# Abolfazlmsl/Oriented-Object-Detection

Hardware: AMD Instinct MI355X
Metric: 416px tiles/sec (whole node), YOLOv11n-OBB 3ch (higher is better)
Workload: dtype f32; 1 GPU; YOLOv11n-OBB 3ch 416x416 tiled inference, single-scale (BASELINE configs[1]): forward + decode + ProbIoU NMS + border filter + per-tile merge + final polygon-IoU merge; step_pipelining=True, nc=12, weights=synthetic seeded, cls bias -8 (no checkpoint offline), final_detections=12170

## Files before the change

### include/obbhip.h

```cpp
#ifndef OBBHIP_H
#define OBBHIP_H

#include <stddef.h>
#include <stdint.h>

#ifdef __cplusplus
extern "C" {
#endif

#define OBB_OK 0
#define OBB_ERR_INVALID (-1)
#define OBB_ERR_HIP (-2)
#define OBB_ERR_STATE (-3)
#define OBB_ERR_FORMAT (-4)

typedef struct obb_ctx obb_ctx;
typedef void *obb_stream_t;

int obb_version(void);
int obb_ctx_create(int device, obb_ctx **out);
int obb_ctx_destroy(obb_ctx *ctx);
const char *obb_last_error(const obb_ctx *ctx);

int obb_set_option(obb_ctx *ctx, const char *key, int64_t value);
// ... 102 lines not shown
int obb_headconv_bwd_geometry(int64_t N, int32_t cin, int32_t cout, int32_t out[4]);
int obb_stemconv_fwd_u8(obb_ctx *ctx, const uint8_t *x, const float *w, int32_t B, int32_t H, int32_t W, int32_t cin, int32_t cout, uint16_t *z,
                        obb_stream_t s);
int obb_stemconv_wgrad_u8(obb_ctx *ctx, const uint8_t *x, const uint16_t *dz, int32_t B, int32_t H, int32_t W, int32_t cin, int32_t cout,
                          float *dw, obb_stream_t s);
int obb_stemconv_wgrad_geometry(int32_t B, int32_t H, int32_t W, int32_t cin, int32_t cout, int32_t out[4]);
int obb_attn_fwd_bf16(obb_ctx *ctx, const uint16_t *qkv, int32_t B, int32_t N, int32_t nh, uint16_t *out, float *lse, obb_stream_t s);
int obb_attn_bwd_bf16(obb_ctx *ctx, const uint16_t *qkv, const uint16_t *out, const float *lse, const uint16_t *dout, const uint16_t *dv_add,
                      int32_t B, int32_t N, int32_t nh, uint16_t *dqkv, obb_stream_t s);
int obb_add_bf16(obb_ctx *ctx, const uint16_t *a, const uint16_t *b, int64_t n, uint16_t *out, obb_stream_t s);
int obb_chanwin_bf16(obb_ctx *ctx, const uint16_t *src, int32_t Cs, int32_t s0, const uint16_t *add, int32_t Ca, int32_t a0, int64_t npix, int32_t n,
                     uint16_t *dst, int32_t Cd, int32_t d0, obb_stream_t s);

int obb_model_load(obb_ctx *ctx, const void *blob_host, size_t bytes);
int obb_model_unload(obb_ctx *ctx, int32_t slot);
int obb_model_info(const obb_ctx *ctx, int32_t h, int32_t w, int32_t *nc, int32_t *ch, int32_t *anchors, int32_t *nconv);
int obb_forward(obb_ctx *ctx, const uint8_t *tiles, int32_t B, int32_t h, int32_t w, float *head, obb_stream_t s);
int obb_forward_gate(obb_ctx *ctx, const uint8_t *tiles, int32_t B, int32_t h, int32_t w, float *head, float *cmax, obb_stream_t s);
int obb_debug_plan(obb_ctx *ctx, int32_t h, int32_t w, char *buf_host, int64_t buf_bytes, int64_t *needed);
int obb_debug_pack_1x1(int32_t form, const float *w, int32_t cout, int32_t cin, int32_t c0, int32_t nc, float *out, int64_t max_floats,
                       int64_t *needed, int32_t *tiling_host);
int obb_debug_activation(obb_ctx *ctx, int32_t h, int32_t w, int32_t B, const char *name, float *out, int64_t max_elems,
                         int64_t *n_elems, int32_t *shape_hwc_host, obb_stream_t s);
int obb_decode_nms(obb_ctx *ctx, const float *head, int32_t B, int32_t h, int32_t w, float conf_thres, float iou_thres,
                   int32_t max_det, float *out, int32_t *count, obb_stream_t s);
int obb_decode_nms_gate(obb_ctx *ctx, const float *head, const float *cmax, int32_t B, int32_t h, int32_t w, float conf_thres, float iou_thres,
                        int32_t max_det, float *det, int32_t *count, obb_stream_t s);
int obb_decode_nms_full(obb_ctx *ctx, const float *head, int32_t B, int32_t h, int32_t w, float conf_thres, float iou_thres,
                        int32_t max_det, float *out, int32_t *count, obb_stream_t s);
int obb_decode(obb_ctx *ctx, const float *head, int32_t B, int32_t h, int32_t w, float *pred, obb_stream_t s);
int obb_probiou_nms(obb_ctx *ctx, const float *boxes, const float *scores, int64_t n, float iou_thres, int32_t *order,
                    uint8_t *keep, obb_stream_t s);
int obb_results(obb_ctx *ctx, const float *det, const float *lb, int64_t n, float *xywhr, float *pts, obb_stream_t s);

int obb_probiou_loss(obb_ctx *ctx, const float *pred, const float *target, const float *weight, int64_t n, float target_scores_sum,
                     float *loss, float *grad_pred, obb_stream_t s);

int obb_tile_labels(obb_ctx *ctx, const double *labels, int64_t n, const int32_t *rects, int32_t ntiles, double min_fraction, uint8_t *mask,
                    double *out, obb_stream_t s);

int obb_dfl_loss(obb_ctx *ctx, const float *pred_dist, const float *target_ltrb, const float *weight, int64_t n, int32_t reg_max,
                 float target_scores_sum, float *loss, float *grad_pred, obb_stream_t s);
int obb_bce_loss(obb_ctx *ctx, const float *logits, const float *targets, int64_t n, float target_scores_sum, float *loss, float *grad_logits,
                 obb_stream_t s);

int obb_crit_decode(obb_ctx *ctx, const void *const *box, int32_t box_bf16, const float *const *cls, const float *const *angle, const int32_t *H,
// ... 51 lines not shown
```

### oriented-object-detection_amd/_lib.py

```python
import ctypes as C
import os

_HERE = os.path.dirname(os.path.abspath(__file__))
SO_PATH = os.path.join(_HERE, "libobbhip.so")
if os.environ.get("OBB_LIB"):
    import sys
    SO_PATH = os.environ["OBB_LIB"]
    sys.stderr.write("oriented_object_detection_amd: OBB_LIB is set -- loading the DIAGNOSTIC library %s instead of the product build\n" % SO_PATH)
_lib = None

c_dp, c_fp, c_ip, c_lp, c_bp = (C.POINTER(C.c_double), C.POINTER(C.c_float), C.POINTER(C.c_int32),
                                C.POINTER(C.c_int64), C.POINTER(C.c_uint8))
_V = C.c_void_p

SIGNATURES = {
    "obb_version": [],
    "obb_ctx_create": [C.c_int, C.POINTER(_V)],
    "obb_ctx_destroy": [_V],
    "obb_last_error": [_V],
    "obb_set_option": [_V, C.c_char_p, C.c_int64],
    "obb_poly_iou_pairs": [_V, _V, _V, C.c_int64, _V, _V],
    "obb_poly_iou_matrix": [_V, _V, _V, C.c_int64, _V, _V, C.c_int64, _V, _V],
    "obb_points_in_quads": [_V, _V, _V, C.c_int64, _V, _V, C.c_int64, _V, _V],
    "obb_build_multich": [_V, _V, C.c_int32, C.c_int32, C.c_int32, _V, _V],
# ... 39 lines not shown
    "obb_headconv_fwd_bf16": [_V, _V, _V, _V, C.c_int64, C.c_int32, C.c_int32, _V, _V],
    "obb_headconv_bwd_bf16": [_V, _V, _V, _V, C.c_int64, C.c_int32, C.c_int32, _V, _V, _V, _V],
    "obb_headconv_bwd_geometry": [C.c_int64, C.c_int32, C.c_int32, c_ip],
    "obb_stemconv_fwd_u8": [_V, _V, _V, C.c_int32, C.c_int32, C.c_int32, C.c_int32, C.c_int32, _V, _V],
    "obb_stemconv_wgrad_u8": [_V, _V, _V, C.c_int32, C.c_int32, C.c_int32, C.c_int32, C.c_int32, _V, _V],
    "obb_stemconv_wgrad_geometry": [C.c_int32, C.c_int32, C.c_int32, C.c_int32, C.c_int32, c_ip],
    "obb_bn_fwd_bf16": [_V, _V, C.c_int64, C.c_int32, _V, _V, C.c_float, C.c_float, _V, _V, _V, _V, _V, C.c_int32, _V],
    "obb_bn_bwd_bf16": [_V, _V, _V, C.c_int64, C.c_int32, _V, _V, _V, _V, _V, _V, _V, C.c_int32, _V],
    "obb_attn_fwd_bf16": [_V, _V, C.c_int32, C.c_int32, C.c_int32, _V, _V, _V],
    "obb_attn_bwd_bf16": [_V, _V, _V, _V, _V, _V, C.c_int32, C.c_int32, C.c_int32, _V, _V],
    "obb_add_bf16": [_V, _V, _V, C.c_int64, _V, _V],
    "obb_chanwin_bf16": [_V, _V, C.c_int32, C.c_int32, _V, C.c_int32, C.c_int32, C.c_int64, C.c_int32, _V, C.c_int32, C.c_int32, _V],
    "obb_gather_tiles": [_V, _V, C.c_int32, C.c_int32, C.c_int32, _V, C.c_int32, C.c_int32, _V, _V],
    "obb_letterbox": [_V, _V, C.c_int32, C.c_int32, C.c_int32, C.c_int32, C.c_int32, C.c_int32, C.c_int32, C.c_int32, _V,
                      C.c_int32, C.c_int32, _V],
    "obb_model_load": [_V, _V, C.c_size_t],
    "obb_model_unload": [_V, C.c_int32],
    "obb_model_info": [_V, C.c_int32, C.c_int32, c_ip, c_ip, c_ip, c_ip],
    "obb_forward": [_V, _V, C.c_int32, C.c_int32, C.c_int32, _V, _V],
    "obb_forward_gate": [_V, _V, C.c_int32, C.c_int32, C.c_int32, _V, _V, _V],
    "obb_debug_plan": [_V, C.c_int32, C.c_int32, C.c_char_p, C.c_int64, c_lp],
    "obb_debug_pack_1x1": [C.c_int32, _V, C.c_int32, C.c_int32, C.c_int32, C.c_int32, _V, C.c_int64, c_lp, c_ip],
    "obb_debug_activation": [_V, C.c_int32, C.c_int32, C.c_int32, C.c_char_p, _V, C.c_int64, c_lp, c_ip, _V],
    "obb_decode_nms": [_V, _V, C.c_int32, C.c_int32, C.c_int32, C.c_float, C.c_float, C.c_int32, _V, _V, _V],
    "obb_decode_nms_gate": [_V, _V, _V, C.c_int32, C.c_int32, C.c_int32, C.c_float, C.c_float, C.c_int32, _V, _V, _V],
    "obb_decode_nms_full": [_V, _V, C.c_int32, C.c_int32, C.c_int32, C.c_float, C.c_float, C.c_int32, _V, _V, _V],
    "obb_decode": [_V, _V, C.c_int32, C.c_int32, C.c_int32, _V, _V],
    "obb_probiou_nms": [_V, _V, _V, C.c_int64, C.c_float, _V, _V, _V],
    "obb_results": [_V, _V, _V, C.c_int64, _V, _V, _V],
    "obb_probiou_loss": [_V, _V, _V, _V, C.c_int64, C.c_float, _V, _V, _V],
    "obb_tile_labels": [_V, _V, C.c_int64, _V, C.c_int32, C.c_double, _V, _V, _V],
    "obb_dfl_loss": [_V, _V, _V, _V, C.c_int64, C.c_int32, C.c_float, _V, _V, _V],
    "obb_bce_loss": [_V, _V, _V, C.c_int64, C.c_float, _V, _V, _V],
    "obb_crit_decode": [_V, _V, C.c_int32, _V, _V, c_ip, c_ip, C.c_int32, C.c_int32, _V, _V, _V, _V, _V],
    "obb_crit_loss": [_V, _V, C.c_int32, _V, _V, c_ip, c_ip, C.c_int32, C.c_int32, _V, _V, _V, c_fp, _V, _V, _V, _V, _V, _V],
    "obb_sgd_step": [_V, _V, _V, _V, C.c_int64, C.c_float, C.c_float, C.c_float, C.c_int32, C.c_int32, _V],
    "obb_adamw_step": [_V, _V, _V, _V, _V, C.c_int64, C.c_int64, C.c_float, C.c_double, C.c_double, C.c_float, C.c_float, _V],
    "obb_grad_sumsq_partials": [c_lp, C.c_int32, c_lp],
    "obb_grad_sumsq": [_V, _V, c_lp, C.c_int32, _V, C.c_int64, _V],
    "obb_clip_coef": [_V, _V, C.c_int64, C.c_double, _V, _V],
    "obb_sgd_step_multi": [_V, _V, _V, _V, c_lp, c_fp, c_fp, C.c_int32, C.c_float, C.c_int32, C.c_int32, _V, _V],
    "obb_adamw_step_multi": [_V, _V, _V, _V, _V, c_lp, c_fp, c_fp, C.c_int32, C.c_int64, C.c_double, C.c_double, C.c_float, _V, _V],
    "obb_grad_accumulate": [_V, _V, _V, c_lp, C.c_int32, C.c_int32, _V],
    "obb_ema_update": [_V, _V, _V, c_lp, C.c_int32, C.c_double, _V],
    "obb_aug_tiles": [_V, _V, C.c_int32, C.c_int32, C.c_int32, _V, C.c_int32, C.c_int32, C.c_int32, _V, _V],
    "obb_aug_labels": [_V, _V, _V, C.c_int32, C.c_int32, _V, C.c_int32, C.c_int32, C.c_double, C.c_double, C.c_double, C.c_int32, _V, _V, _V, _V, _V],
# ... 40 lines not shown
```

### oriented-object-detection_amd/csrc/ctx.h

```cpp
#pragma once
#include <hip/hip_runtime.h>

#include <cstdarg>
#include <cstdint>
#include <cstdio>
#include <map>
#include <memory>
#include <string>
#include <vector>

#include "../../include/obbhip.h"

namespace obb {
struct Model;
struct EngineOpts {
    bool tail = true, tail16 = true, bneck = true, bneck_cv2 = true, c3kimg = true, dwpw = true, upfold = true, stem = true, front = true, pair = true, hmerge = true,
         sppf_fuse = true, attn_mfma = true, xtile = true, nitile = true, nc2 = true, blk32 = true, c3k2f = true, pw32 = true, upacc = true, graph = true;
    int fwd_split = 0 , microbatch = 1024;
};
}

struct obb_ctx {
    int device = 0;
    std::string err;
    struct Slot { void *p = nullptr; size_t bytes = 0; };
    std::vector<Slot> ws;
    std::shared_ptr<obb::Model> model;
    std::map<int, std::shared_ptr<obb::Model>> slots;
    int slot = 0;
    bool opt_f16 = true;
    bool opt_f32 = false;
    obb::EngineOpts opt;
    void *workspace(int slot, size_t bytes);
    ~obb_ctx();
};

namespace obb {
int set_error(obb_ctx *ctx, int code, const char *fmt, ...);
extern thread_local std::string g_tls_error;

// ... 20 lines not shown
```

### oriented-object-detection_amd/csrc/engine.hip

```cpp
#include <algorithm>
#include <cmath>
#include <cstdlib>
#include <cstring>

#include "plan.h"

namespace obb {

static int ensure_capacity(obb_ctx *ctx, Plan &P, int B) {
    if (B <= P.cap) return OBB_OK;
    int cap = std::max(B, 1);
    int64_t off = 0;
    for (Buf &b : P.bufs) {
        b.off = off;
        if (b.virt) continue;
        off += ((int64_t)cap * b.per_img() * (b.f32 ? 4 : 2) + 255) / 256 * 256;
    }
    void *slab = nullptr;
    OBB_HIP(ctx, hipDeviceSynchronize());
    P.drop_graphs();
    if (P.slab) { (void)hipFree(P.slab); P.slab = nullptr; P.cap = 0; }
    OBB_HIP(ctx, hipMalloc(&slab, (size_t)off + 256));
    P.slab = slab;
    P.cap = cap;
// ... 206 lines not shown
                                    float *__restrict__ dst, int blk, int64_t ps) {
    int64_t i = (int64_t)blockIdx.x * 256 + threadIdx.x;
    int64_t total = (int64_t)B * npix_per_img * C;
    if (i >= total) return;
    int c = (int)(i % C) + co;
    int64_t pix = (i / C) % npix_per_img;
    int64_t b = i / ((int64_t)C * npix_per_img);
    dst[i] = HX<F16>::one(blk > 0 ? src[(int64_t)(c / blk) * ps + b * bs + pix * blk + c % blk] : src[b * bs + pix * cs + c]);
}

__global__ void k_f32_slice_copy(const float *__restrict__ src, int64_t bs, int cs, int co, int C, int64_t npix_per_img, int B, float *__restrict__ dst, int blk) {
    int64_t i = (int64_t)blockIdx.x * 256 + threadIdx.x;
    if (i >= (int64_t)B * npix_per_img * C) return;
    int c = (int)(i % C) + co;
    int64_t pix = (i / C) % npix_per_img;
    int64_t b = i / ((int64_t)C * npix_per_img);
    dst[i] = blk > 0 ? src[b * bs + (int64_t)(c / blk) * npix_per_img * blk + pix * blk + c % blk] : src[b * bs + pix * cs + c];
}

static bool *switch_of(obb_ctx *ctx, const std::string &k) {
    struct { const char *key; bool *flag; } sw[] = {
        {"tail", &ctx->opt.tail}, {"tail16", &ctx->opt.tail16}, {"bneck", &ctx->opt.bneck}, {"bneck_cv2", &ctx->opt.bneck_cv2},
        {"c3kimg", &ctx->opt.c3kimg}, {"dwpw", &ctx->opt.dwpw}, {"upfold", &ctx->opt.upfold}, {"stem", &ctx->opt.stem}, {"front", &ctx->opt.front}, {"pair", &ctx->opt.pair},
        {"hmerge", &ctx->opt.hmerge}, {"sppf_fuse", &ctx->opt.sppf_fuse}, {"attn_mfma", &ctx->opt.attn_mfma}, {"xtile", &ctx->opt.xtile}, {"nitile", &ctx->opt.nitile}, {"nc2", &ctx->opt.nc2}, {"blk32", &ctx->opt.blk32}, {"c3k2f", &ctx->opt.c3k2f}, {"pw32", &ctx->opt.pw32}, {"upacc", &ctx->opt.upacc}, {"graph", &ctx->opt.graph}};
    for (auto &e : sw)
        if (k == e.key) return e.flag;
    return nullptr;
}

}

using namespace obb;

extern "C" {

int obb_model_load(obb_ctx *ctx, const void *blob_host, size_t bytes) {
    OBB_REQUIRE(ctx, ctx && blob_host && bytes > 0, "obb_model_load: bad arguments");
    OBB_HIP(ctx, hipSetDevice(ctx->device));
    OBB_HIP(ctx, hipDeviceSynchronize());
    std::shared_ptr<Model> M(new Model());
    M->blob.assign((const char *)blob_host, (const char *)blob_host + bytes);
    int rc = parse_blob(ctx, *M);
    if (rc) return rc;
    M->f16 = ctx->opt_f16;
    M->f32 = ctx->opt_f32;
    M->o = ctx->opt;
    M->o.hmerge = M->o.tail && M->o.hmerge;
// ... 163 lines not shown
                const int ni = (!op.one_d && ctx->model->o.nitile) ? conv_ni_supported(L) : 1;
                snprintf(line, sizeof line, "conv %s k%d s%d cin%d cout%d out%dx%d TH%d TW%d MF%d NF%d CK%d NI%d gx%d gy%d lds%d macs%.0f\n", op.name.c_str(), L.ks,
                         L.stride, L.cin, L.cout, op.Ho, op.Wo, ni > 1 ? op.Ho : L.TH, ni > 1 ? op.Wo : L.TW, L.MF, L.NF, L.CK, ni, grid_x, grid_y, (int)conv_lds_bytes(L), op.macs);
                break;
            }
            case OP_DW: snprintf(line, sizeof line, "dwconv %s c%d out%dx%d macs%.0f\n", op.name.c_str(), op.in.C, op.Ho, op.Wo, op.macs); break;
            case OP_C3KIMG: snprintf(line, sizeof line, "c3kimg %s c%d out%dx%d macs%.0f\n", op.name.c_str(), op.in.C, op.Ho, op.Wo, op.macs); break;
            case OP_DWPW: snprintf(line, sizeof line, "dwpw %s c%d tail%d out%dx%d macs%.0f\n", op.name.c_str(), op.dwpw.cin, op.dwpw.tail_cout, op.Ho, op.Wo, op.macs); break;
            case OP_BNECK: snprintf(line, sizeof line, "bneck %s c%d co%d out%dx%d rows4 macs%.0f\n", op.name.c_str(), op.bneck.C, op.bneck.CO, op.Ho, op.Wo, op.macs); break;
            case OP_SPPF: snprintf(line, sizeof line, "pool %s c%d out%dx%d x3 macs0\n", op.name.c_str(), op.in.C, op.Ho, op.Wo); break;
            case OP_POOL: snprintf(line, sizeof line, "pool %s c%d out%dx%d macs0\n", op.name.c_str(), op.in.C, op.Ho, op.Wo); break;
            case OP_UP: snprintf(line, sizeof line, "upsample %s c%d out%dx%d macs0\n", op.name.c_str(), op.in.C, op.Ho, op.Wo); break;
            case OP_PW32:
                snprintf(line, sizeof line, "pw32 %s k1 s1 cin%d cout%d out%dx%d waves%d raw%d lds%d macs%.0f\n", op.name.c_str(), op.pw32.cin, op.pw32.cout, op.Ho, op.Wo,
                         op.pw32.cin * 256 <= 80 * 1024 ? 8 : 16, op.pw32.raw ? 1 : 0, op.pw32.cin * 256, op.macs);
                break;
            case OP_C3K2F32: {
                int th, tw;
                c3k2f32_tile(op.H, op.W, th, tw);
                snprintf(line, sizeof line, "c3k2f32 %s c%d co%d out%dx%d TH%d TW%d macs%.0f\n", op.name.c_str(), op.c3k2f.C, op.c3k2f.CO, op.Ho, op.Wo, th, tw, op.macs);
                break;
            }
            case OP_STEM32:
                snprintf(line, sizeof line, "stem32 %s k3 s2 cin%d cout%d out%dx%d rows%d macs%.0f\n", op.name.c_str(), op.stem32.cin, op.stem32.cout, op.Ho, op.Wo, 4, op.macs);
                break;
            case OP_STEM:
                snprintf(line, sizeof line, "stem %s k3 s2 cin%d cout%d out%dx%d rows%d macs%.0f\n", op.name.c_str(), op.stem.cin, op.stem.cout, op.Ho, op.Wo, 4, op.macs);
                break;
            case OP_FRONT: snprintf(line, sizeof line, "front %s cin%d out%dx%d macs%.0f\n", op.name.c_str(), op.front.cin, op.Ho, op.Wo, op.macs); break;
            case OP_ATTN: snprintf(line, sizeof line, "attn %s N%d nh%d macs%.0f\n", op.name.c_str(), op.N, op.nh, op.macs); break;
        }
        out += line;
    }
    snprintf(line, sizeof line, "total_macs %.0f bytes_per_img %lld nbufs %zu nops %zu\n", P->macs_per_img, (long long)P->bytes_per_img, P->bufs.size(),
             P->ops.size());
    out += line;
    *needed = (int64_t)out.size() + 1;
    if (buf && buf_bytes >= *needed) memcpy(buf, out.c_str(), out.size() + 1);
    return OBB_OK;
}

int obb_debug_activation(obb_ctx *ctx, int32_t h, int32_t w, int32_t B, const char *name, float *out, int64_t max_elems,
                         int64_t *n_elems, int32_t *shape_hwc_host, obb_stream_t s) {
    OBB_REQUIRE(ctx, ctx && name && n_elems, "obb_debug_activation: bad arguments");
    Plan *P = nullptr;
    int rc = get_plan(ctx, h, w, &P);
    if (rc) return rc;
// ... 2 lines not shown
    OBB_REQUIRE(ctx, B <= P->cap, "obb_debug_activation: run obb_forward with B >= %d first", B);
    const Slice &sl = it->second;
    const Buf &b = P->bufs[sl.buf];
    int64_t n = (int64_t)B * b.H * b.W * sl.C;
    *n_elems = n;
    if (shape_hwc_host) { shape_hwc_host[0] = b.H; shape_hwc_host[1] = b.W; shape_hwc_host[2] = sl.C; }
    if (!out) return OBB_OK;
    OBB_REQUIRE(ctx, max_elems >= n, "obb_debug_activation: output too small (%lld < %lld)", (long long)max_elems, (long long)n);
    const int64_t hw = (int64_t)b.H * b.W;
    const int64_t d_bs = b.blk > 0 ? hw * b.blk : b.per_img(), d_ps = b.blk > 0 ? (int64_t)P->cap * hw * b.blk : 0;
    if (b.f32)
        hipLaunchKernelGGL(k_f32_slice_copy, dim3((unsigned)cdiv(n, 256)), dim3(256), 0, (hipStream_t)s, (const float *)b.p, (int64_t)b.per_img(), b.C, sl.co, sl.C, hw,
                           B, out, b.blk32);
    else if (ctx->model->f16)
        hipLaunchKernelGGL(k_half_slice_to_f32<true>, dim3((unsigned)cdiv(n, 256)), dim3(256), 0, (hipStream_t)s, (const bf16_t *)b.p, d_bs, b.C,
                           sl.co, sl.C, hw, B, out, b.blk, d_ps);
    else
        hipLaunchKernelGGL(k_half_slice_to_f32<false>, dim3((unsigned)cdiv(n, 256)), dim3(256), 0, (hipStream_t)s, (const bf16_t *)b.p, d_bs, b.C,
                           sl.co, sl.C, hw, B, out, b.blk, d_ps);
    OBB_LAUNCH_CHECK(ctx);
    return OBB_OK;
}

}
```

### oriented-object-detection_amd/csrc/f32path.h

```cpp
#pragma once
#include <hip/hip_runtime.h>

#include <cstdint>
#include <vector>

#include "tensorref.h"

namespace obb {

struct Conv32Tiling { int TH, TW, CK, WC, MFM, NI, NC; };

struct Conv32Launch {
    TensorRef in, out, res;
    const float *wpk = nullptr;
    const float *bias = nullptr;
    const float *lut = nullptr;
    int B = 0, Hin = 0, Win = 0, Hout = 0, Wout = 0;
    int cin = 0, cout = 0, ks = 1, stride = 1, act = 1, in_u8 = 0, flip_bgr = 0;
    int out_hw = 0;
    TensorRef in2;
    int up_c = 0, up_W = 0, up_HW = 0;
    TensorRef acc_init;
    const float *tail_w = nullptr;
    const float *tail_b = nullptr;
// ... 5 lines not shown
    int TH = 1, TW = 208, CK = 16, WC = 4, MFM = 7;
    int dw = 0, dw_act = 1;
    int NI = 1;
    int tiles_y = 1, tiles_x = 1;
    int NC = 1;
    int xtile = 1;
    void set_tiling(const Conv32Tiling &t) { TH = t.TH; TW = t.TW; CK = t.CK; WC = t.WC; MFM = t.MFM; NI = t.NI; NC = t.NC; }
};

Conv32Tiling plan_conv32(int ks, int stride, int cin, int cout, int Hout, int Wout, bool in_u8, bool vcat = false, bool nc2 = false);
bool conv32_tail_supported(const Conv32Tiling &t, int cout1, int cout2);
Conv32Tiling plan_dwpw32(int cin, int cout, int H, int W);
std::vector<float> pack_dwpw32_weights(const float *pw_oihw, int cout, int cin, const float *dw_c9, const float *dw_bias, const Conv32Tiling &t);
std::vector<float> pack_conv32_weights(const float *w_oihw, int cout, int cin, int ks, const Conv32Tiling &t, const int *cout_perm, bool in_u8);
size_t conv32_lds_bytes(const Conv32Launch &L);
hipError_t launch_conv32(const Conv32Launch &L, hipStream_t st);

struct Stem32Launch {
    const uint8_t *in = nullptr;
    TensorRef out;
    const float *wpk = nullptr;
    const float *bias = nullptr, *lut = nullptr;
    int B = 0, Hin = 0, Win = 0, cin = 3, cout = 16, act = 1;
};
bool stem32_supported(int cin, int cout, int ks, int stride, int Hin, int Win);
std::vector<float> pack_stem32_weights(const float *w_oihw, int cout, int cin, bool flip_bgr);
hipError_t launch_stem32(const Stem32Launch &L, hipStream_t st);

hipError_t launch_dwconv3_f32(const TensorRef &in, const TensorRef &out, const TensorRef &res, const float *w9c, const float *bias, int B, int H, int W,
                              int C, int act, hipStream_t st);
hipError_t launch_maxpool5_f32(const TensorRef &in, const TensorRef &out, int B, int H, int W, int C, hipStream_t st);
hipError_t launch_upsample2_f32(const TensorRef &in, const TensorRef &out, int B, int H, int W, int C, hipStream_t st);
hipError_t launch_sppf_pools_f32(const TensorRef &cat, int B, int H, int W, int C, hipStream_t st);
hipError_t launch_attention_f32(const TensorRef &qkv, const TensorRef &out, int B, int N, int nh, int kd, int hd, bool use_mfma, hipStream_t st);

}
```

### oriented-object-detection_amd/csrc/f32path.hip

```cpp
#include "f32path.h"
#include "c32geom.h"
#include "c32params.h"
#include "launchcfg.h"

#include <algorithm>
#include <cmath>
#include <cstdlib>
#include <cstring>

namespace obb {

typedef __attribute__((ext_vector_type(4))) float f32x4;
typedef __attribute__((ext_vector_type(4))) unsigned int u32x4;

__device__ __forceinline__ float silu32(float x) { return x * __builtin_amdgcn_rcpf(1.0f + __expf(-x)); }

template <int KS, int MFM, int WC, int NW, bool IN_U8, bool VCAT, int TAIL, bool DW = false, int NC = 1, bool BLK = false, bool AINIT = false>
__global__ __launch_bounds__(NW * 64, NW / 2) void k_conv_f32(const C32Params P) {
    static_assert(NW == c32::kNW, "the planner and the launch checks size tiles for c32::kNW waves");
    static_assert(!AINIT || (KS == 1 && NC == 2 && !VCAT), "accumulator init: the 1-D 1x1 two-fragment form only");
    static_assert(NC == 1 || (NC == 2 && TAIL == 0 && !DW && !IN_U8), "two cout fragments per wave: plain / VCAT forms only");
    extern __shared__ __attribute__((aligned(16))) char smem[];
    constexpr int SKS = DW ? 3 : KS;
    constexpr int NT = NW * 64, WP = NW / WC, PAD = SKS / 2;
    const int tid = threadIdx.x, lane = tid & 63;
    const int wave = __builtin_amdgcn_readfirstlane(tid >> 6);
    const int g = lane >> 4, pl = lane & 15;
    const int wc = wave % WC, wp = wave / WC;
    const int xcd = blockIdx.x & 7, lin = blockIdx.x >> 3;
    const int cb = lin % P.ncb;
    int t = (lin / P.ncb) * 8 + xcd;
// ... 639 lines not shown
            for (int nf = 0; nf < NF; ++nf) {
                acc0[nf] = __builtin_amdgcn_mfma_f32_16x16x4f32(wA[nf][t], b0[t], acc0[nf], 0, 0, 0);
                acc1[nf] = __builtin_amdgcn_mfma_f32_16x16x4f32(wA[nf][t], b1[t], acc1[nf], 0, 0, 0);
            }
        }
#pragma unroll
        for (int h = 0; h < 2; ++h) {
            if (h == 1 && !two) break;
            float *op = orow + (int64_t)(16 * (f0 + h) + j) * P.out_cs;
#pragma unroll
            for (int nf = 0; nf < NF; ++nf) {
                const f32x4 a = h ? acc1[nf] : acc0[nf];
                float v[4] = {a[0] + bv[nf].x, a[1] + bv[nf].y, a[2] + bv[nf].z, a[3] + bv[nf].w};
                if (P.act) {
#pragma unroll
                    for (int q = 0; q < 4; ++q) v[q] = silu32(v[q]);
                }
                *reinterpret_cast<float4 *>(op + nf * 16) = make_float4(v[0], v[1], v[2], v[3]);
            }
        }
    }
}

static int stem32_rs(int Win, int cin) { return (4 + Win * cin + 3) & ~3; }

bool stem32_supported(int cin, int cout, int ks, int stride, int Hin, int Win) {
    if (ks != 3 || stride != 2 || (cin != 3 && cin != 4) || (cout != 16 && cout != 32)) return false;
    if (Hin % 8 || Win % 32) return false;
    return (size_t)(9 * stem32_rs(Win, cin) + 256) * 4 <= 64 * 1024 && 9 * Win * cin / 4 <= 16 * 256;
}

hipError_t launch_stem32(const Stem32Launch &L, hipStream_t st) {
    if (!stem32_supported(L.cin, L.cout, 3, 2, L.Hin, L.Win) || L.out.cpb || (L.out.cs & 3) || (L.out.co & 3) || !L.lut) return hipErrorInvalidValue;
    Stem32Params P;
    P.in = L.in; P.in_bs = (int64_t)L.Hin * L.Win * L.cin;
    P.out = (float *)L.out.p; P.out_bs = L.out.bs; P.out_cs = L.out.cs; P.out_co = L.out.co;
    P.wA = L.wpk; P.bias = L.bias; P.lut = L.lut;
    P.Hin = L.Hin; P.Win = L.Win; P.Hout = L.Hin / 2; P.Wout = L.Win / 2; P.act = L.act; P.RS = stem32_rs(L.Win, L.cin);
    const size_t lds = (size_t)(9 * P.RS + 256) * 4;
    const dim3 grid((unsigned)(L.B * (P.Hout / 4)));
    if (L.cin == 3 && L.cout == 16) hipLaunchKernelGGL((k_stem_f32<3, 1>), grid, dim3(256), lds, st, P);
    else if (L.cin == 4 && L.cout == 16) hipLaunchKernelGGL((k_stem_f32<4, 1>), grid, dim3(256), lds, st, P);
    else if (L.cin == 3 && L.cout == 32) hipLaunchKernelGGL((k_stem_f32<3, 2>), grid, dim3(256), lds, st, P);
    else hipLaunchKernelGGL((k_stem_f32<4, 2>), grid, dim3(256), lds, st, P);
    return hipGetLastError();
}

__global__ __launch_bounds__(256) void k_dwconv3_f32(TensorRef in, TensorRef out, TensorRef res, const float *__restrict__ w, const float *__restrict__ bias,
                                                    int B, int H, int W, int C, int act) {
    const int c4n = C >> 2;
    const int64_t idx = (int64_t)blockIdx.x * 256 + threadIdx.x;
    if (idx >= (int64_t)B * H * W * c4n) return;
    const int c4 = (int)(idx % c4n);
    const int64_t pix = idx / c4n;
    const int x = (int)(pix % W), y = (int)((pix / W) % H), b = (int)(pix / ((int64_t)W * H));
    const float *ip = (const float *)in.p + (int64_t)b * in.bs + in.co + c4 * 4;
// ... 344 lines not shown
```

### oriented-object-detection_amd/csrc/netplan.hip

```cpp
#include <algorithm>
#include <cmath>
#include <cstring>

#include "plan.h"

namespace obb {

#pragma pack(push, 1)
struct BlobHeader { char magic[4]; uint32_t version, nrec; int32_t nc, ch; float width, depth; int32_t max_ch, reg_max; char scale[8]; };
struct BlobRec { char name[64]; int32_t c1, c2, k, s, g, act; uint64_t w_off, b_off; };
#pragma pack(pop)

int parse_blob(obb_ctx *ctx, Model &M) {
    const size_t n = M.blob.size();
    if (n < sizeof(BlobHeader)) return set_error(ctx, OBB_ERR_FORMAT, "weight blob too small (%zu bytes)", n);
    BlobHeader H;
    memcpy(&H, M.blob.data(), sizeof H);
    if (memcmp(H.magic, "OBBW", 4) != 0 || H.version != 1) return set_error(ctx, OBB_ERR_FORMAT, "bad weight blob magic/version");
    if (H.reg_max != kRegMax) return set_error(ctx, OBB_ERR_FORMAT, "reg_max %d unsupported", H.reg_max);
    if (H.ch != 3 && H.ch != 4) return set_error(ctx, OBB_ERR_FORMAT, "input channels %d unsupported (3 or 4)", H.ch);
    if (H.nc < 1 || H.nc > 1024) return set_error(ctx, OBB_ERR_FORMAT, "nc %d out of range", H.nc);
    M.nc = H.nc; M.ch = H.ch; M.width = H.width; M.depth = H.depth; M.max_ch = H.max_ch;
    M.scale = std::string(H.scale, strnlen(H.scale, 8));
    size_t tbl = sizeof(BlobHeader);
// ... 174 lines not shown
            err = set_error(ctx, OBB_ERR_STATE, "layer %s cannot read the channel-blocked buffer '%s'", name.c_str(), P.bufs[in.buf].name.c_str());
            return;
        }
        if (M.f32 && ((res.C && P.bufs[res.buf].blk32) || (tail_name && out.buf >= 0 && P.bufs[out.buf].blk32))) {
            err = set_error(ctx, OBB_ERR_STATE, "layer %s: residual / fused-1x1 output in a channel-blocked buffer", name.c_str());
            return;
        }
        if (op.vin && !perm && !tail_name && head_level < 0 && !res.C && upacc_ok(r, P.bufs[in.buf], Hin, Win)) return emit_upacc(op, r);
        if (M.f32 && M.o.pw32 && r->k == 1 && !in_u8 && !op.vin && !tail_name && head_level < 0 && !P.bufs[in.buf].blk32 && pw32_supported(cin, r->c2) &&
            !(res.C && P.bufs[res.buf].blk32))
            return emit_pw32(op, r, perm);
        if (M.f32) return emit_conv32(op, r, perm, tail_name);
        if (stem_in && stem_supported(cin, r->c2, r->k, r->s, Hin, Win) && r->act && stem_scale_is_exact(M.f16)) return emit_stem16(op, r);
        emit_conv16(op, r, perm, tail_name);
    }

    void emit_stem32(Op op, const ConvRecord *r) {
        op.type = OP_STEM32;
        Stem32Launch &S = op.stem32;
        S.Hin = op.H; S.Win = op.W; S.cin = r->c1; S.cout = r->c2; S.act = r->act;
        S.wpk = upload(pack_stem32_weights(r->w, r->c2, r->c1, M.ch == 3));
        S.bias = bias_padded(r);
        S.lut = M.lut32_dev;
        emit(op, r->name, op.out);
    }
    void emit_pw32(Op op, const ConvRecord *r, const int *perm) {
        op.type = OP_PW32;
        Pw32Launch &L = op.pw32;
        L.cin = r->c1; L.cout = r->c2; L.act = r->act;
        L.wpk = upload(pack_pw32_weights(r->w, r->c2, r->c1, perm));
        L.bias = bias_padded(r, perm);
        emit(op, r->name, op.out);
    }
    bool upacc_ok(const ConvRecord *r, const Buf &vb, int H, int W) const {
        if (!M.f32 || !M.o.upacc || !M.o.pw32 || !M.o.nc2 || r->k != 1 || vb.va_C % 16 || (H & 1) || (W & 1) || P.bufs[vb.va_buf].blk32) return false;
        if (!pw32_supported(vb.va_C, r->c2) || vb.vb_C < 64 || r->c2 % 32) return false;
        const Conv32Tiling t = plan_conv32(1, 1, vb.vb_C, r->c2, H, W, false, false, true);
        return t.NC == 2 && t.WC == 2 && t.MFM == 3 && vb.vb_C % t.CK == 0;
    }
    void emit_upacc(Op op, const ConvRecord *r) {
        const Buf vb = P.bufs[op.in.buf];
        const int up_c = vb.va_C, sk = vb.vb_C, Hc = op.H / 2, Wc = op.W / 2;
        const int part = buf(Hc, Wc, r->c2, r->name + ".up", true);
        Op oc;
        oc.type = OP_PW32; oc.name = r->name + ".up"; oc.in = Slice{vb.va_buf, vb.va_co, up_c}; oc.out = whole(part);
        oc.H = oc.Ho = Hc; oc.W = oc.Wo = Wc; oc.one_d = true;
// ... 525 lines not shown
```

### oriented-object-detection_amd/ops.py

```python
import ctypes as C
import contextlib
import ctypes as _ct
import os
from typing import List, Optional

import torch

from . import _lib

_ctx = {}
T = torch.Tensor


def ctx(device=None):
    idx = torch.cuda.current_device() if device is None else torch.device(device).index or 0
    if idx not in _ctx:
        h = C.c_void_p()
        _lib.check(_lib.lib().obb_ctx_create(idx, C.byref(h)))
        _ctx[idx] = h
    return _ctx[idx]


def destroy_contexts():
    for h in _ctx.values():
# ... 1066 lines not shown
def records_to_dets(records, n, rects, strike_cls=1):
    rec = _chk(records, torch.int32, "records")
    r = _chk(rects, torch.int32, "rects").reshape(-1, 4)
    n = int(n)
    gb = torch.empty((n, 8), dtype=torch.float64, device=rec.device)
    c = torch.empty(n, dtype=torch.int32, device=rec.device)
    f = torch.empty(n, dtype=torch.float64, device=rec.device)
    a = torch.empty(n, dtype=torch.float64, device=rec.device)
    if n:
        _O.records_to_dets(rec, n, r, int(strike_cls), gb, c, f, a)
    return gb, c, f, a


def gather_compact(recv):
    r = _chk(recv, torch.int32, "recv")
    world, cap = r.shape[0], r.shape[1] - 1
    out = torch.empty((world * cap, 12), dtype=torch.int32, device=r.device)
    counts = torch.empty(world + 1, dtype=torch.int32, device=r.device)
    _O.gather_compact(r, out, counts)
    return out, counts


PRECISIONS = {"f16": 16, "fp16": 16, "bf16": 1016, "f32": 32, "fp32": 32}
MODEL_OPTIONS = ("fuse", "tail", "tail16", "bneck", "bneck_cv2", "c3kimg", "dwpw", "upfold", "stem", "front", "pair", "hmerge", "sppf_fuse", "attn_mfma", "xtile", "nitile", "nc2", "blk32", "c3k2f", "pw32", "upacc", "graph")


def select_model(slot, device=None):
    _call("obb_set_option", ctx(device), b"model_slot", int(slot))


def get_option(key, device=None):
    v = C.c_int64(0)
    _call("obb_get_option", ctx(device), key.encode(), C.byref(v))
    return v.value


@contextlib.contextmanager
def engine_state(device=None):
    keys = ("precision",) + MODEL_OPTIONS[1:]
    c = ctx(device)
    slot, saved = get_option("model_slot", device), {k: get_option(k, device) for k in keys}
    try:
        yield
    finally:
        for k, v in saved.items():
            _call("obb_set_option", c, k.encode(), v)
        _call("obb_set_option", c, b"model_slot", slot)
# ... 59 lines not shown
        return hd
    out = torch.zeros(hd.shape[:-1] + ((no + 3) // 4 * 4,), dtype=hd.dtype, device=hd.device)
    out[..., :no] = hd
    return out


def debug_plan(h, w, device=None):
    c = ctx(device)
    need = C.c_int64(0)
    _call("obb_debug_plan", c, h, w, None, 0, C.byref(need))
    buf = C.create_string_buffer(need.value)
    _call("obb_debug_plan", c, h, w, buf, need.value, C.byref(need))
    return buf.value.decode().strip().split("\n")


def debug_activation(name, B, h, w, device=None):
    c = ctx(device)
    n = C.c_int64(0)
    shp = (C.c_int32 * 3)()
    _call("obb_debug_activation", c, h, w, B, name.encode(), None, 0, C.byref(n), shp, _stream())
    out = torch.empty((B, shp[0], shp[1], shp[2]), dtype=torch.float32, device=torch.device("cuda", torch.cuda.current_device()))
    _O.debug_activation(name, B, h, w, out)
    return out


def decode(head, h, w):
    hd = _padded_head(_chk(head, torch.float32, "head"))
    B, A, _ = hd.shape
    pred = torch.empty((B, A, 4 + model_info(h, w, hd.device)["nc"] + 1), dtype=torch.float32, device=hd.device)
    _O.decode(hd, h, w, pred)
    return pred


def decode_nms(head, h, w, conf=0.25, iou=0.7, max_det=300, full=False, zero=True, cmax=None):
    hd = _padded_head(_chk(head, torch.float32, "head"))
    B = hd.shape[0]
    det = (torch.zeros if zero or not B else torch.empty)((B, max_det, 7), dtype=torch.float32, device=hd.device)
    count = (torch.zeros if zero or not B else torch.empty)(B, dtype=torch.int32, device=hd.device)
    if B and cmax is not None and not full:
        cm = _chk(cmax, torch.float32, "cmax")
        if tuple(cm.shape) != tuple(hd.shape[:2]):
            raise ValueError("decode_nms: cmax must be [B, A] of the same head")
        _O.decode_nms_gate(hd, cm, h, w, float(conf), float(iou), int(max_det), det, count)
    elif B:
        (_O.decode_nms_full if full else _O.decode_nms)(hd, h, w, float(conf), float(iou), int(max_det), det, count)
    return det, count
# ... 383 lines not shown
```

Baseline: 33130 tiles/s.

## Add persistent double-buffered walking stem32 kernel with u8 LDS image

Result: no change. 33280 tiles/s (median of 6 runs) (+0.4%).

```diff
diff --git a/include/obbhip.h b/include/obbhip.h
--- a/include/obbhip.h
+++ b/include/obbhip.h
@@ -148,6 +148,8 @@
                        int64_t *needed, int32_t *tiling_host);
 int obb_debug_activation(obb_ctx *ctx, int32_t h, int32_t w, int32_t B, const char *name, float *out, int64_t max_elems,
                          int64_t *n_elems, int32_t *shape_hwc_host, obb_stream_t s);
+int obb_debug_stem32(obb_ctx *ctx, const uint8_t *tiles, int32_t B, int32_t h, int32_t w, int32_t cin, int32_t cout, const float *w_oihw_host,
+                     const float *bias_host, int32_t act, int32_t walk, float *out, int32_t out_cs, int32_t out_co, int32_t *walked, obb_stream_t s);
 int obb_decode_nms(obb_ctx *ctx, const float *head, int32_t B, int32_t h, int32_t w, float conf_thres, float iou_thres,
                    int32_t max_det, float *out, int32_t *count, obb_stream_t s);
 int obb_decode_nms_gate(obb_ctx *ctx, const float *head, const float *cmax, int32_t B, int32_t h, int32_t w, float conf_thres, float iou_thres,
diff --git a/oriented-object-detection_amd/_lib.py b/oriented-object-detection_amd/_lib.py
--- a/oriented-object-detection_amd/_lib.py
+++ b/oriented-object-detection_amd/_lib.py
@@ -85,6 +85,7 @@
     "obb_debug_plan": [_V, C.c_int32, C.c_int32, C.c_char_p, C.c_int64, c_lp],
     "obb_debug_pack_1x1": [C.c_int32, _V, C.c_int32, C.c_int32, C.c_int32, C.c_int32, _V, C.c_int64, c_lp, c_ip],
     "obb_debug_activation": [_V, C.c_int32, C.c_int32, C.c_int32, C.c_char_p, _V, C.c_int64, c_lp, c_ip, _V],
+    "obb_debug_stem32": [_V, _V, C.c_int32, C.c_int32, C.c_int32, C.c_int32, C.c_int32, _V, _V, C.c_int32, C.c_int32, _V, C.c_int32, C.c_int32, c_ip, _V],
     "obb_decode_nms": [_V, _V, C.c_int32, C.c_int32, C.c_int32, C.c_float, C.c_float, C.c_int32, _V, _V, _V],
     "obb_decode_nms_gate": [_V, _V, _V, C.c_int32, C.c_int32, C.c_int32, C.c_float, C.c_float, C.c_int32, _V, _V, _V],
     "obb_decode_nms_full": [_V, _V, C.c_int32, C.c_int32, C.c_int32, C.c_float, C.c_float, C.c_int32, _V, _V, _V],
diff --git a/oriented-object-detection_amd/csrc/ctx.h b/oriented-object-detection_amd/csrc/ctx.h
--- a/oriented-object-detection_amd/csrc/ctx.h
+++ b/oriented-object-detection_amd/csrc/ctx.h
@@ -15,7 +15,7 @@
 struct Model;
 struct EngineOpts {
     bool tail = true, tail16 = true, bneck = true, bneck_cv2 = true, c3kimg = true, dwpw = true, upfold = true, stem = true, front = true, pair = true, hmerge = true,
-         sppf_fuse = true, attn_mfma = true, xtile = true, nitile = true, nc2 = true, blk32 = true, c3k2f = true, pw32 = true, upacc = true, graph = true;
+         sppf_fuse = true, attn_mfma = true, xtile = true, nitile = true, nc2 = true, blk32 = true, c3k2f = true, pw32 = true, upacc = true, stemwalk = true, graph = true;
     int fwd_split = 0 , microbatch = 1024;
 };
 }
diff --git a/oriented-object-detection_amd/csrc/engine.hip b/oriented-object-detection_amd/csrc/engine.hip
--- a/oriented-object-detection_amd/csrc/engine.hip
+++ b/oriented-object-detection_amd/csrc/engine.hip
@@ -252,7 +252,7 @@
     struct { const char *key; bool *flag; } sw[] = {
         {"tail", &ctx->opt.tail}, {"tail16", &ctx->opt.tail16}, {"bneck", &ctx->opt.bneck}, {"bneck_cv2", &ctx->opt.bneck_cv2},
         {"c3kimg", &ctx->opt.c3kimg}, {"dwpw", &ctx->opt.dwpw}, {"upfold", &ctx->opt.upfold}, {"stem", &ctx->opt.stem}, {"front", &ctx->opt.front}, {"pair", &ctx->opt.pair},
-        {"hmerge", &ctx->opt.hmerge}, {"sppf_fuse", &ctx->opt.sppf_fuse}, {"attn_mfma", &ctx->opt.attn_mfma}, {"xtile", &ctx->opt.xtile}, {"nitile", &ctx->opt.nitile}, {"nc2", &ctx->opt.nc2}, {"blk32", &ctx->opt.blk32}, {"c3k2f", &ctx->opt.c3k2f}, {"pw32", &ctx->opt.pw32}, {"upacc", &ctx->opt.upacc}, {"graph", &ctx->opt.graph}};
+        {"hmerge", &ctx->opt.hmerge}, {"sppf_fuse", &ctx->opt.sppf_fuse}, {"attn_mfma", &ctx->opt.attn_mfma}, {"xtile", &ctx->opt.xtile}, {"nitile", &ctx->opt.nitile}, {"nc2", &ctx->opt.nc2}, {"blk32", &ctx->opt.blk32}, {"c3k2f", &ctx->opt.c3k2f}, {"pw32", &ctx->opt.pw32}, {"upacc", &ctx->opt.upacc}, {"stemwalk", &ctx->opt.stemwalk}, {"graph", &ctx->opt.graph}};
     for (auto &e : sw)
         if (k == e.key) return e.flag;
     return nullptr;
@@ -462,7 +462,7 @@
                 break;
             }
             case OP_STEM32:
-                snprintf(line, sizeof line, "stem32 %s k3 s2 cin%d cout%d out%dx%d rows%d macs%.0f\n", op.name.c_str(), op.stem32.cin, op.stem32.cout, op.Ho, op.Wo, 4, op.macs);
+                snprintf(line, sizeof line, "stem32 %s k3 s2 cin%d cout%d out%dx%d rows%d walk%d macs%.0f\n", op.name.c_str(), op.stem32.cin, op.stem32.cout, op.Ho, op.Wo, 4, op.stem32.walk, op.macs);
                 break;
             case OP_STEM:
                 snprintf(line, sizeof line, "stem %s k3 s2 cin%d cout%d out%dx%d rows%d macs%.0f\n", op.name.c_str(), op.stem.cin, op.stem.cout, op.Ho, op.Wo, 4, op.macs);
@@ -511,4 +511,29 @@
     return OBB_OK;
 }
 
-}
+int obb_debug_stem32(obb_ctx *ctx, const uint8_t *tiles, int32_t B, int32_t h, int32_t w, int32_t cin, int32_t cout, const float *w_oihw_host,
+                     const float *bias_host, int32_t act, int32_t walk, float *out, int32_t out_cs, int32_t out_co, int32_t *walked, obb_stream_t s) {
+    OBB_REQUIRE(ctx, ctx && tiles && w_oihw_host && bias_host && out && B >= 1, "obb_debug_stem32: bad arguments");
+    OBB_REQUIRE(ctx, stem32_supported(cin, cout, 3, 2, h, w), "obb_debug_stem32: no fp32 stem kernel for cin %d cout %d at %d x %d", cin, cout, h, w);
+    OBB_REQUIRE(ctx, out_co >= 0 && out_co + cout <= out_cs, "obb_debug_stem32: channels [%d, %d) outside a %d-channel buffer", out_co, out_co + cout, out_cs);
+    OBB_HIP(ctx, hipSetDevice(ctx->device));
+    std::vector<float> host = pack_stem32_weights(w_oihw_host, cout, cin, cin == 3);
+    const size_t nw = host.size();
+    host.insert(host.end(), bias_host, bias_host + cout);
+    for (int v = 0; v < 256; ++v) host.push_back((float)v / 255.0f);
+    float *dev = nullptr;
+    OBB_HIP(ctx, hipMalloc((void **)&dev, host.size() * 4));
+    hipError_t e = hipMemcpy(dev, host.data(), host.size() * 4, hipMemcpyHostToDevice);
+    Stem32Launch L;
+    L.in = tiles; L.B = B; L.Hin = h; L.Win = w; L.cin = cin; L.cout = cout; L.act = act; L.walk = walk;
+    L.wpk = dev; L.bias = dev + nw; L.lut = dev + nw + cout;
+    L.out.p = out; L.out.cs = out_cs; L.out.co = out_co; L.out.bs = (int64_t)(h / 2) * (w / 2) * out_cs;
+    if (walked) *walked = stem32_walks(L) ? 1 : 0;
+    if (e == hipSuccess) e = launch_stem32(L, (hipStream_t)s);
+    if (e == hipSuccess) e = hipStreamSynchronize((hipStream_t)s);
+    (void)hipFree(dev);
+    OBB_HIP(ctx, e);
+    return OBB_OK;
+}
+
+}
diff --git a/oriented-object-detection_amd/csrc/f32path.h b/oriented-object-detection_amd/csrc/f32path.h
--- a/oriented-object-detection_amd/csrc/f32path.h
+++ b/oriented-object-detection_amd/csrc/f32path.h
@@ -51,8 +51,10 @@
     const float *wpk = nullptr;
     const float *bias = nullptr, *lut = nullptr;
     int B = 0, Hin = 0, Win = 0, cin = 3, cout = 16, act = 1;
+    int walk = 1;
 };
 bool stem32_supported(int cin, int cout, int ks, int stride, int Hin, int Win);
+bool stem32_walks(const Stem32Launch &L);
 std::vector<float> pack_stem32_weights(const float *w_oihw, int cout, int cin, bool flip_bgr);
 hipError_t launch_stem32(const Stem32Launch &L, hipStream_t st);
 
diff --git a/oriented-object-detection_amd/csrc/f32path.hip b/oriented-object-detection_amd/csrc/f32path.hip
--- a/oriented-object-detection_amd/csrc/f32path.hip
+++ b/oriented-object-detection_amd/csrc/f32path.hip
@@ -7,6 +7,7 @@
 #include <cmath>
 #include <cstdlib>
 #include <cstring>
+#include <type_traits>
 
 namespace obb {
 
@@ -692,7 +693,164 @@
     }
 }
 
+struct StemWalkParams {
+    const uint8_t *in;
+    float *out; int64_t out_bs; int out_cs, out_co;
+    const float *wA, *bias, *lut;
+    int Win, Wout, act, RS, stripes, nitems, nwalk;
+};
+
+template <int CIN, int NF, bool U8>
+__global__ __launch_bounds__(512, U8 ? 4 : 2) void k_stem_walk_f32(const StemWalkParams P) {
+    using ET = typename std::conditional<U8, uint8_t, float>::type;
+    extern __shared__ __attribute__((aligned(16))) float sst[];
+    constexpr int K = 9 * CIN, KST = (K + 3) / 4, NR = 9, NT = 512;
+    constexpr int MAXC = 2;
+    constexpr int MARG = 16 / (int)sizeof(ET);
+    const int tid = threadIdx.x, lane = tid & 63, wave = __builtin_amdgcn_readfirstlane(tid >> 6);
+    const int g = lane >> 4, j = lane & 15;
+    const int it0 = (int)((int64_t)blockIdx.x * P.nitems / P.nwalk), it1 = (int)(((int64_t)blockIdx.x + 1) * P.nitems / P.nwalk);
+    if (it0 >= it1) return;
+    float *slut = sst;
+    ET *img = reinterpret_cast<ET *>(sst + 256);
+    const int RS = P.RS, ibuf = NR * RS, rowb = P.Win * CIN, cpr = rowb >> 4;
+    if (tid < 256) slut[tid] = P.lut[tid];
+    if (tid < 2 * NR) *reinterpret_cast<u32x4 *>(img + tid * RS) = u32x4{0u, 0u, 0u, 0u};
+    __syncthreads();
+    auto put = [&](ET *dst, const u32x4 v) {
+        if constexpr (U8) *reinterpret_cast<u32x4 *>(dst) = v;
+        else {
+#pragma unroll
+            for (int q = 0; q < 4; ++q)
+                *reinterpret_cast<float4 *>(dst + 4 * q) = make_float4(slut[v[q] & 255u], slut[(v[q] >> 8) & 255u], slut[(v[q] >> 16) & 255u], slut[v[q] >> 24]);
+        }
+    };
+    int bn = it0 / P.stripes, sn = it0 - bn * P.stripes;
+    for (int c = tid; c < cpr; c += NT) {
+        u32x4 v = {0u, 0u, 0u, 0u};
+        if (sn > 0) v = *reinterpret_cast<const u32x4 *>(P.in + ((int64_t)it0 * 8 - 1) * rowb + c * 16);
+        put(img + ibuf + MARG + 16 * c, v);
+    }
+    int goff[MAXC], loff[MAXC];
+    bool ok[MAXC];
+#pragma unroll
+    for (int k = 0; k < MAXC; ++k) {
+        const int i = tid + k * NT;
+        ok[k] = i < 8 * cpr;
+        const int ic = min(i, 8 * cpr - 1), lr = ic / cpr, d = ic - lr * cpr;
+        goff[k] = lr * rowb + 16 * d;
+        loff[k] = (lr + 1) * RS + MARG + 16 * d;
+    }
+    float wA[NF][KST];
+    int koff[KST];
+#pragma unroll
+    for (int t = 0; t < KST; ++t) {
+        const int k = 4 * t + g;
+        const int tap = k / CIN, c = k - tap * CIN;
+        const int ky = tap / 3, kx = tap - ky * 3;
+        koff[t] = (MARG - CIN) + (k < K ? ky * RS + kx * CIN + c : 0);
+#pragma unroll
+        for (int nf = 0; nf < NF; ++nf) wA[nf][t] = P.wA[(nf * KST + t) * 64 + lane];
+    }
+    float4 bv[NF];
+#pragma unroll
+    for (int nf = 0; nf < NF; ++nf) bv[nf] = *reinterpret_cast<const float4 *>(P.bias + nf * 16 + 4 * g);
+    const int r = wave >> 1, nfr = P.Wout >> 4, n0 = (nfr + 1) >> 1;
+    const int fa = (wave & 1) ? n0 : 0, fb = (wave & 1) ? nfr : n0;
+
+    auto mma = [&](const ET *cur, const int f0, const bool two, f32x4 (&acc0)[NF], f32x4 (&acc1)[NF]) {
+        const int pb0 = 2 * r * RS + 2 * (16 * f0 + j) * CIN, pb1 = two ? pb0 + 32 * CIN : pb0;
+#pragma unroll
+        for (int nf = 0; nf < NF; ++nf) { acc0[nf] = f32x4{0.f, 0.f, 0.f, 0.f}; acc1[nf] = f32x4{0.f, 0.f, 0.f, 0.f}; }
+        float b0[KST], b1[KST];
+        if constexpr (U8) {
+            unsigned q0[KST], q1[KST];
+#pragma unroll
+            for (int t = 0; t < KST; ++t) { q0[t] = cur[pb0 + koff[t]]; q1[t] = cur[pb1 + koff[t]]; }
+#pragma unroll
+            for (int t = 0; t < KST; ++t) { b0[t] = slut[q0[t]]; b1[t] = slut[q1[t]]; }
+        } else {
+#pragma unroll
+            for (int t = 0; t < KST; ++t) { b0[t] = cur[pb0 + koff[t]]; b1[t] = cur[pb1 + koff[t]]; }
+        }
+#pragma unroll
+        for (int t = 0; t < KST; ++t) {
+#pragma unroll
+            for (int nf = 0; nf < NF; ++nf) {
+                acc0[nf] = __builtin_amdgcn_mfma_f32_16x16x4f32(wA[nf][t], b0[t], acc0[nf], 0, 0, 0);
+                acc1[nf] = __builtin_amdgcn_mfma_f32_16x16x4f32(wA[nf][t], b1[t], acc1[nf], 0, 0, 0);
+            }
+        }
+    };
+    auto store = [&](float *orow, const int f0, const bool two, const f32x4 (&acc0)[NF], const f32x4 (&acc1)[NF]) {
+#pragma unroll
+        for (int h = 0; h < 2; ++h) {
+            if (h == 1 && !two) break;
+            float *op = orow + (int64_t)(16 * (f0 + h) + j) * P.out_cs;
+#pragma unroll
+            for (int nf = 0; nf < NF; ++nf) {
+                const f32x4 a = h ? acc1[nf] : acc0[nf];
+                float v[4] = {a[0] + bv[nf].x, a[1] + bv[nf].y, a[2] + bv[nf].z, a[3] + bv[nf].w};
+                if (P.act) {
+#pragma unroll
+                    for (int q = 0; q < 4; ++q) v[q] = silu32(v[q]);
+                }
+                *reinterpret_cast<float4 *>(op + nf * 16) = make_float4(v[0], v[1], v[2], v[3]);
+            }
+        }
+    };
+
+    int p = 0, b = 0, s = 0;
+    for (int it = it0 - 1; it < it1; ++it) {
+        const bool have = it >= it0, more = it + 1 < it1;
+        const uint8_t *src = P.in + (int64_t)(more ? it + 1 : it) * 8 * rowb;
+        u32x4 wv[MAXC];
+#pragma unroll
+        for (int k = 0; k < MAXC; ++k) wv[k] = *reinterpret_cast<const u32x4 *>(src + goff[k]);
+        ET *cur = img + p * ibuf, *nxt = img + (p ^ 1) * ibuf;
+        f32x4 acc0[NF], acc1[NF];
+        float *orow = nullptr;
+        int fl = fa;
+        bool any = false, two = false;
+        if (have) {
+            if (more) {
+                const int nvec = cpr * (int)sizeof(ET);
+                for (int c = tid; c < nvec; c += NT) {
+                    u32x4 v = {0u, 0u, 0u, 0u};
+                    if (sn != 0) v = *reinterpret_cast<const u32x4 *>(cur + 8 * RS + MARG + c * MARG);
+                    *reinterpret_cast<u32x4 *>(nxt + MARG + c * MARG) = v;
+                }
+            }
+            orow = P.out + (int64_t)b * P.out_bs + (int64_t)(4 * s + r) * P.Wout * P.out_cs + P.out_co + 4 * g;
+            for (; fl + 2 < fb; fl += 2) {
+                mma(cur, fl, true, acc0, acc1);
+                store(orow, fl, true, acc0, acc1);
+            }
+            any = fl < fb;
+            two = fl + 1 < fb;
+            if (any) mma(cur, fl, two, acc0, acc1);
+        }
+        if (more) {
+#pragma unroll
+            for (int k = 0; k < MAXC; ++k)
+                if (ok[k]) put(nxt + loff[k], wv[k]);
+        }
+        if (any) store(orow, fl, two, acc0, acc1);
+        __syncthreads();
+        p ^= 1; b = bn; s = sn;
+        if (++sn == P.stripes) { sn = 0; ++bn; }
+    }
+}
+
+#ifdef OBB_STEMWALK_F32IMG
+constexpr bool kStemWalkU8 = false;
+#else
+constexpr bool kStemWalkU8 = true;
+#endif
+
 static int stem32_rs(int Win, int cin) { return (4 + Win * cin + 3) & ~3; }
+static int stemwalk_rs(int Win, int cin) { return kStemWalkU8 ? (16 + Win * cin + 15) & ~15 : stem32_rs(Win, cin); }
+static size_t stemwalk_lds(int Win, int cin) { return 1024 + (size_t)2 * 9 * stemwalk_rs(Win, cin) * (kStemWalkU8 ? 1 : 4); }
 
 bool stem32_supported(int cin, int cout, int ks, int stride, int Hin, int Win) {
     if (ks != 3 || stride != 2 || (cin != 3 && cin != 4) || (cout != 16 && cout != 32)) return false;
@@ -700,8 +858,40 @@
     return (size_t)(9 * stem32_rs(Win, cin) + 256) * 4 <= 64 * 1024 && 9 * Win * cin / 4 <= 16 * 256;
 }
 
+bool stem32_walks(const Stem32Launch &L) {
+    return L.walk && stem32_supported(L.cin, L.cout, 3, 2, L.Hin, L.Win) && ((uintptr_t)L.in & 15) == 0 && L.Win * L.cin <= 2 * 512 * 16 &&
+           stemwalk_lds(L.Win, L.cin) <= 128 * 1024;
+}
+
+template <int CIN, int NF>
+static hipError_t launch_stem_walk(const Stem32Launch &L, hipStream_t st) {
+    const void *fn = (const void *)k_stem_walk_f32<CIN, NF, kStemWalkU8>;
+    const size_t lds = stemwalk_lds(L.Win, L.cin);
+    int n = 0, ncu = 0;
+    hipError_t e;
+    if ((e = allow_dyn_lds(fn, 128 * 1024)) != hipSuccess) return e;
+    if ((e = resident_blocks(fn, 512, lds, &n)) != hipSuccess || (e = cu_count(&ncu)) != hipSuccess) return e;
+    StemWalkParams P;
+    P.in = L.in;
+    P.out = (float *)L.out.p; P.out_bs = L.out.bs; P.out_cs = L.out.cs; P.out_co = L.out.co;
+    P.wA = L.wpk; P.bias = L.bias; P.lut = L.lut;
+    P.Win = L.Win; P.Wout = L.Win / 2; P.act = L.act; P.RS = stemwalk_rs(L.Win, L.cin); P.stripes = L.Hin / 8;
+    const int64_t items = (int64_t)L.B * P.stripes;
+    if (items < 1 || items >= (1ll << 31)) return hipErrorInvalidValue;
+    P.nitems = (int)items;
+    P.nwalk = (int)std::min<int64_t>(items, (int64_t)std::max(1, n) * std::max(1, ncu));
+    hipLaunchKernelGGL((k_stem_walk_f32<CIN, NF, kStemWalkU8>), dim3((unsigned)P.nwalk), dim3(512), lds, st, P);
+    return hipGetLastError();
+}
+
 hipError_t launch_stem32(const Stem32Launch &L, hipStream_t st) {
     if (!stem32_supported(L.cin, L.cout, 3, 2, L.Hin, L.Win) || L.out.cpb || (L.out.cs & 3) || (L.out.co & 3) || !L.lut) return hipErrorInvalidValue;
+    if (stem32_walks(L)) {
+        if (L.cin == 3 && L.cout == 16) return launch_stem_walk<3, 1>(L, st);
+        if (L.cin == 4 && L.cout == 16) return launch_stem_walk<4, 1>(L, st);
+        if (L.cin == 3 && L.cout == 32) return launch_stem_walk<3, 2>(L, st);
+        return launch_stem_walk<4, 2>(L, st);
+    }
     Stem32Params P;
     P.in = L.in; P.in_bs = (int64_t)L.Hin * L.Win * L.cin;
     P.out = (float *)L.out.p; P.out_bs = L.out.bs; P.out_cs = L.out.cs; P.out_co = L.out.co;
diff --git a/oriented-object-detection_amd/csrc/netplan.hip b/oriented-object-detection_amd/csrc/netplan.hip
--- a/oriented-object-detection_amd/csrc/netplan.hip
+++ b/oriented-object-detection_amd/csrc/netplan.hip
@@ -220,6 +220,7 @@
         S.wpk = upload(pack_stem32_weights(r->w, r->c2, r->c1, M.ch == 3));
         S.bias = bias_padded(r);
         S.lut = M.lut32_dev;
+        S.walk = M.o.stemwalk ? 1 : 0;
         emit(op, r->name, op.out);
     }
     void emit_pw32(Op op, const ConvRecord *r, const int *perm) {
diff --git a/oriented-object-detection_amd/ops.py b/oriented-object-detection_amd/ops.py
--- a/oriented-object-detection_amd/ops.py
+++ b/oriented-object-detection_amd/ops.py
@@ -1112,7 +1112,7 @@
 
 
 PRECISIONS = {"f16": 16, "fp16": 16, "bf16": 1016, "f32": 32, "fp32": 32}
-MODEL_OPTIONS = ("fuse", "tail", "tail16", "bneck", "bneck_cv2", "c3kimg", "dwpw", "upfold", "stem", "front", "pair", "hmerge", "sppf_fuse", "attn_mfma", "xtile", "nitile", "nc2", "blk32", "c3k2f", "pw32", "upacc", "graph")
+MODEL_OPTIONS = ("fuse", "tail", "tail16", "bneck", "bneck_cv2", "c3kimg", "dwpw", "upfold", "stem", "front", "pair", "hmerge", "sppf_fuse", "attn_mfma", "xtile", "nitile", "nc2", "blk32", "c3k2f", "pw32", "upacc", "stemwalk", "graph")
 
 
 def select_model(slot, device=None):
@@ -1218,6 +1218,20 @@
     out = torch.empty((B, shp[0], shp[1], shp[2]), dtype=torch.float32, device=torch.device("cuda", torch.cuda.current_device()))
     _O.debug_activation(name, B, h, w, out)
     return out
+
+
+def debug_stem32(tiles, w, bias, out, out_co=0, act=True, walk=True):
+    import numpy as np
+    t, o = _chk(tiles, torch.uint8, "tiles"), _chk(out, torch.float32, "out")
+    B, h, ww, cin = t.shape
+    wh, bh = np.ascontiguousarray(w, np.float32), np.ascontiguousarray(bias, np.float32)
+    cout = wh.shape[0]
+    if wh.shape != (cout, cin, 3, 3) or bh.shape != (cout,) or o.dim() != 4 or tuple(o.shape[:3]) != (B, h // 2, ww // 2):
+        raise ValueError("debug_stem32: w must be [cout,cin,3,3], bias [cout], out [B,h/2,w/2,C]")
+    walked = C.c_int32(-1)
+    _call("obb_debug_stem32", ctx(t.device), _p(t), B, h, ww, cin, cout, wh.ctypes.data_as(C.c_void_p), bh.ctypes.data_as(C.c_void_p), 1 if act else 0,
+          1 if walk else 0, _p(o), o.shape[3], int(out_co), C.byref(walked), _stream())
+    return bool(walked.value)
 
 
 def decode(head, h, w):
```
